# lammps/lammps-plugins

Measured on AMD Instinct MI355X. Metric: Matom-steps/sec, higher is better.
Workload: dtype f64; 1 GPU; REBO-MoS bulk: in.rebomos-bulk cell replicated 24x24x24; atoms=3981312, style=rebomos, parallelism=spatial-dd1, transport=none (one GPU), rccl_library_is_test_double=False, thermo_every=10, displacement_check=every step, deferred on-device flag, dangerous_builds=0, inner_skin=adaptive from 1.0, late_style_list_builds_rank0=0, row_prunings_late_rank0=0, rccl_ranks=1

## Files before the change

lammps-plugins_amd/csrc/domain.hip:

```cpp
#include "mdp_common.h"

#include <rocprim/rocprim.hpp>

#include <cmath>

namespace {

__device__ __forceinline__ void dd_shift_cart(const DdGeom &G, const double s0, const double s1, const double s2,
                                              double out[3])
{
  out[0] = G.h[0] * s0 + G.h[5] * s1 + G.h[4] * s2;
  out[1] = G.h[1] * s1 + G.h[3] * s2;
  out[2] = G.h[2] * s2;
}

__device__ __forceinline__ unsigned dd_cell10(const double u)
{
  int g = (int) (u * 1024.0);
  g = g < 0 ? 0 : (g > 1023 ? 1023 : g);
  return (unsigned) g;
}

template <bool IMAGE>
__global__ __launch_bounds__(256) void dd_remap_kernel(const DdGeom G, const int n, double4 *__restrict__ xq,
// ... 426 lines not shown
  D.nghost_old = c->nghost;
  mdp_tally_drop(c);
  MDP_HIP(c, D.dest.reserve((size_t) n + 1));
  MDP_HIP(c, hipMemsetAsync(D.counters.p, 0, sizeof(int) * (4 * G.nranks + 16), st));
  if (n && c->image_set) dd_remap_kernel<true><<<nblk(n), 256, 0, st>>>(G, n, c->xq.p, D.dest.p, D.counters.p, c->image.p);
  else if (n) dd_remap_kernel<false><<<nblk(n), 256, 0, st>>>(G, n, c->xq.p, D.dest.p, D.counters.p, nullptr);
  MDP_HIP(c, hipGetLastError());
  MDP_TRY(mdp_read_one(c, D.counters.p, sizeof(int) * G.nranks, D.mig_send.data()));
  D.mig_send[G.rank] = 0;
  D.mig_total = 0;
  for (int q = 0; q < G.nranks; q++) D.mig_total += D.mig_send[q];
  if (send_counts)
    for (int q = 0; q < G.nranks; q++) send_counts[q] = D.mig_send[q];
  return MDP_OK;
}

int mdp_dd_migrate_pack(mdp_ctx *c, double *d_buf)
{
  MDP_TRY(dd_require(c));
  MdpDomain &D = c->dd;
  const DdGeom &G = D.G;
  hipStream_t st = c->stream;
  if (!D.mig_total) return MDP_OK;
  if (!d_buf) return mdp_fail(c, MDP_EINVAL, "mdp_dd_migrate_pack: no buffer for %d leaving atoms", D.mig_total);
  std::vector<int> off(2 * (size_t) G.nranks, 0);
  for (int q = 1; q < G.nranks; q++) off[q] = off[q - 1] + D.mig_send[q - 1];
  int *seg = D.counters.p + G.nranks, *cur = D.counters.p + 2 * G.nranks;
  MDP_TRY(mdp_write_small(c, seg, off.data(), sizeof(int) * 2 * G.nranks));
  const int *mask = c->mask_set ? c->mask.p : nullptr;
  if (c->image_set)
    dd_pack_leavers_kernel<true><<<nblk(D.nlocal_old), 256, 0, st>>>(D.nlocal_old, G.rank, D.dest.p, seg, cur, c->xq.p, c->v.p,
                                                                     c->type.p, c->tag.p, mask, c->image.p, d_buf);
  else
    dd_pack_leavers_kernel<false><<<nblk(D.nlocal_old), 256, 0, st>>>(D.nlocal_old, G.rank, D.dest.p, seg, cur, c->xq.p, c->v.p,
                                                                      c->type.p, c->tag.p, mask, nullptr, d_buf);
  MDP_HIP(c, hipGetLastError());
  MDP_HIP(c, hipStreamSynchronize(st));
  return MDP_OK;
}

int mdp_dd_migrate_end(mdp_ctx *c, int narrive, const double *d_buf)
{
  MDP_TRY(dd_require(c));
  MdpDomain &D = c->dd;
  const DdGeom &G = D.G;
  hipStream_t st = c->stream;
  if (narrive < 0 || (narrive > 0 && !d_buf)) return mdp_fail(c, MDP_EINVAL, "mdp_dd_migrate_end: bad arrival buffer");
  const int nold = D.nlocal_old, ntot = nold + narrive, nnew = ntot - D.mig_total;
  if ((long long) ntot >= (1ll << 29)) return mdp_fail(c, MDP_EINVAL, "too many atoms for NEIGHMASK");
  MDP_HIP(c, c->xq.reserve((size_t) ntot + 1, true, st));
  MDP_HIP(c, c->v.reserve((size_t) 3 * ntot + 3, true, st));
  MDP_HIP(c, c->type.reserve((size_t) ntot + 32, true, st));
  MDP_HIP(c, c->tag.reserve((size_t) ntot + 1, true, st));
  MDP_HIP(c, D.dest.reserve((size_t) ntot + 1, true, st));
  if (c->mask_set) MDP_HIP(c, c->mask.reserve((size_t) ntot + 1, true, st));
  if (c->image_set) MDP_HIP(c, c->image.reserve((size_t) ntot + 1, true, st));
  MDP_HIP(c, c->mass_type.reserve(32));
  MDP_HIP(c, hipMemcpyAsync(c->mass_type.p, c->h_mass, sizeof(double) * 16, hipMemcpyHostToDevice, st));
  int *d_map = D.counters.p + 3 * G.nranks;
  MDP_HIP(c, hipMemcpyAsync(d_map, c->map, sizeof(int) * 16, hipMemcpyHostToDevice, st));
  if (narrive)
    dd_unpack_arrivals_kernel<<<nblk(narrive), 256, 0, st>>>(narrive, nold, d_buf, d_map, c->xq.p, c->v.p, c->type.p,
                                                             c->tag.p, c->mask_set ? c->mask.p : nullptr,
                                                             c->image_set ? c->image.p : nullptr, D.dest.p, G.rank);
  MDP_HIP(c, D.key_a.reserve((size_t) ntot + 1));
  MDP_HIP(c, D.key_b.reserve((size_t) ntot + 1));
  MDP_HIP(c, D.idx_a.reserve((size_t) ntot + 1));
  MDP_HIP(c, D.idx_b.reserve((size_t) ntot + 1));
  const size_t room = (size_t) nnew + (size_t) D.nghost_old + (size_t) D.nghost_old / 16;
  MDP_HIP(c, D.xq_tmp.reserve(room + 1));
  MDP_HIP(c, D.v_tmp.reserve((size_t) 3 * nnew + 3));
  MDP_HIP(c, D.type_tmp.reserve(room + 32));
  MDP_HIP(c, D.tag_tmp.reserve(room + 1));
  if (c->mask_set) MDP_HIP(c, D.mask_tmp.reserve((size_t) nnew + 1));
  if (c->image_set) MDP_HIP(c, D.image_tmp.reserve((size_t) nnew + 1));
  MDP_HIP(c, c->rmass.reserve((size_t) nnew + 1));
  if (ntot) {
    const int shell_last = c->cfg.style == 2;
    dd_order_key_kernel<<<nblk(ntot), 256, 0, st>>>(G, ntot, c->xq.p, c->tag.p, D.dest.p, D.key_a.p, D.idx_a.p,
                                                    shell_last);
    MDP_HIP(c, hipGetLastError());
    MDP_TRY(sort_u64(c, D.key_a.p, D.key_b.p, D.idx_a.p, D.idx_b.p, (size_t) ntot, 64));
    if (c->cfg.style == 1) {
      MDP_TRY(mdp_chunk_by_element(c, ntot, nnew, D.idx_b.p, D.idx_a.p, c->xq.p, nullptr, nullptr));
      D.idx_a.swap(D.idx_b);
    }
  }
  if (nnew) {
    dd_permute_kernel<<<nblk(nnew), 256, 0, st>>>(nnew, D.idx_b.p, c->xq.p, c->v.p, c->type.p, c->tag.p, c->mass_type.p,
                                                  D.xq_tmp.p, D.v_tmp.p, D.type_tmp.p, D.tag_tmp.p, c->rmass.p,
                                                  c->mask_set ? c->mask.p : nullptr, c->mask_set ? D.mask_tmp.p : nullptr,
                                                  c->image_set ? c->image.p : nullptr, c->image_set ? D.image_tmp.p : nullptr);
    MDP_HIP(c, hipGetLastError());
  }
  c->xq.swap(D.xq_tmp);
  c->v.swap(D.v_tmp);
  c->type.swap(D.type_tmp);
  c->tag.swap(D.tag_tmp);
  if (c->mask_set) {
    c->mask.swap(D.mask_tmp);
    c->mask_n = nnew;
  }
  if (c->image_set) c->image.swap(D.image_tmp);
  c->nlocal = nnew;
  c->nghost = 0;
  c->nall = nnew;
  c->cfg.nlocal = nnew;
  c->neigh_set = false;
  c->rebo_packed = false;
  return MDP_OK;
}

int mdp_dd_borders_begin(mdp_ctx *c, int *send_counts)
{
  MDP_TRY(dd_require(c));
  MdpDomain &D = c->dd;
  const DdGeom &G = D.G;
  hipStream_t st = c->stream;
  const int n = c->nlocal;
  MDP_HIP(c, D.ent_cnt.reserve((size_t) n + 2));
  MDP_HIP(c, D.ent_off.reserve((size_t) n + 2));
  int nent = 0;
  if (n) {
    dd_border_kernel<false><<<nblk(n), 256, 0, st>>>(G, n, c->xq.p, D.ent_cnt.p, nullptr, nullptr, nullptr, nullptr);
    MDP_HIP(c, hipGetLastError());
    MDP_TRY(mdp_scan_exclusive_int(c, D.ent_cnt.p, D.ent_off.p, n));
    MDP_TRY(mdp_read_one(c, D.ent_off.p + n, sizeof(int), &nent));
  }
  D.nent = nent;
  const int ncls = G.nranks + 1;
  std::vector<int> start(ncls, -1);
  if (nent) {
    MDP_HIP(c, D.ent_atom.reserve((size_t) nent));
    MDP_HIP(c, D.ent_code.reserve((size_t) nent));
    MDP_HIP(c, D.key_a.reserve((size_t) nent));
    MDP_HIP(c, D.key_b.reserve((size_t) nent));
    MDP_HIP(c, D.idx_a.reserve((size_t) nent));
    MDP_HIP(c, D.idx_b.reserve((size_t) nent));
    dd_border_kernel<true><<<nblk(n), 256, 0, st>>>(G, n, c->xq.p, nullptr, D.ent_off.p, D.ent_atom.p, D.ent_code.p,
                                                    D.key_a.p);
    MDP_HIP(c, hipGetLastError());
    MDP_HIP(c, rocprim::transform(rocprim::counting_iterator<int>(0), D.idx_a.p, (size_t) nent,
                                  [] __device__(int v) -> int { return v; }, st));
    int bits = 33;
    while ((1ll << (bits - 32)) < ncls + 1) bits++;
    MDP_TRY(sort_u64(c, D.key_a.p, D.key_b.p, D.idx_a.p, D.idx_b.p, (size_t) nent, bits));
    int *d_start = D.counters.p + 3 * G.nranks + 16;
    MDP_HIP(c, hipMemsetAsync(d_start, 0xFF, sizeof(int) * ncls, st));
    dd_class_start_kernel<<<nblk(nent), 256, 0, st>>>(nent, D.key_b.p, d_start);
    MDP_HIP(c, hipGetLastError());
    MDP_TRY(mdp_read_one(c, d_start, sizeof(int) * ncls, start.data()));
  }
  std::vector<int> cnt(ncls, 0);
  int next = nent;
  for (int k = ncls - 1; k >= 0; k--)
    if (start[k] >= 0) {
      cnt[k] = next - start[k];
      next = start[k];
    }
  D.nself = cnt[0];
  D.nsend = nent - D.nself;
  for (int q = 0; q < G.nranks; q++) D.bord_send[q] = cnt[q + 1];
  if (D.bord_send[G.rank] != 0 && !G.self_remote)
    return mdp_fail(c, MDP_EINVAL, "dd: internal error (self entries in the send list)");
  MDP_HIP(c, c->ghost_owner.reserve((size_t) D.nself + 1));
  MDP_HIP(c, c->ghost_shift.reserve((size_t) 3 * D.nself + 3));
  MDP_HIP(c, D.sendlist.reserve((size_t) D.nsend + 1));
// ... 215 lines not shown
```

lammps-plugins_amd/csrc/mdp_api.hip:

```cpp
#include "mdp_common.h"

#include <rocprim/rocprim.hpp>

#include <condition_variable>
#include <functional>
#include <mutex>
#include <thread>
#include <unistd.h>

#include <cmath>

void mdp_rebomos_fill_dev(mdp_ctx *c, double skin);

int mdp_fail(mdp_ctx *c, int code, const char *fmt, ...)
{
  char buf[1024];
  va_list ap;
  va_start(ap, fmt);
  vsnprintf(buf, sizeof buf, fmt, ap);
  va_end(ap);
  if (c) c->err = buf;
  return code;
}

// ... 502 lines not shown
  nt = nt > W.width() ? W.width() : nt;
  if (nt <= 1) {
    for (size_t k = 0; k < n; k++) dst[k] += src[k];
    return;
  }
  const size_t chunk = ((n + nt - 1) / nt + 7) & ~(size_t) 7;
  W.run(nt, [=](unsigned t) {
    const size_t b = t * chunk, e = b + chunk < n ? b + chunk : n;
    for (size_t k = b; k < e; k++) dst[k] += src[k];
  });
}

int mdp_host_download_add(mdp_ctx *c, double *h_dst, double *h_stage, const double *d_src, size_t n)
{
  hipStream_t st = c->stream;
  size_t cut[MDP_DOWN_CHUNKS + 1];
  int nch = 1;
  cut[0] = 0;
  cut[1] = n;
  if (n > (1u << 21)) {
    const size_t per = ((n + MDP_DOWN_CHUNKS - 1) / MDP_DOWN_CHUNKS + 7) & ~(size_t) 7;
    nch = MDP_DOWN_CHUNKS;
    for (int k = 1; k <= nch; k++) cut[k] = (size_t) k * per < n ? (size_t) k * per : n;
  }
  if (!c->ev_down[0])
    for (int k = 0; k < MDP_DOWN_CHUNKS; k++) MDP_HIP(c, hipEventCreateWithFlags(&c->ev_down[k], hipEventDisableTiming));
  for (int k = 0; k < nch; k++) {
    const size_t b = cut[k], e = cut[k + 1];
    if (b >= e) continue;
    MDP_HIP(c, hipMemcpyAsync(h_stage + b, d_src + b, sizeof(double) * (e - b), hipMemcpyDeviceToHost, st));
    MDP_HIP(c, hipEventRecord(c->ev_down[k], st));
  }
  for (int k = 0; k < nch; k++) {
    const size_t b = cut[k], e = cut[k + 1];
    if (b >= e) continue;
    MDP_HIP(c, hipEventSynchronize(c->ev_down[k]));
    mdp_host_add(h_dst + b, h_stage + b, e - b);
  }
  return MDP_OK;
}

int mdp_pack_xq(mdp_ctx *c, const double *d_x3, const int *d_type, int count)
{
  static_assert(sizeof(double4) == 32, "double4 layout");
  const int n = count >= 0 ? count : c->nall;
  if (n <= 0) return MDP_OK;
  int *d_map = nullptr;
  if (d_type) {
    d_map = c->type.p + c->nall;
  }
  if (c->host_sort)
    pack_xq_perm_kernel<<<nblk(n), 256, 0, c->stream>>>(n, d_x3, d_type, d_map, c->host_perm.p, c->xq.p);
  else
    pack_xq_kernel<<<nblk(n), 256, 0, c->stream>>>(n, d_x3, d_type, d_map, c->xq.p);
  MDP_HIP(c, hipGetLastError());
  return MDP_OK;
}

static int host_sort_atoms(mdp_ctx *c)
{
  const int nall = c->nall;
  const char *e = getenv("MDP_HOST_SORT");
  const bool own_lists = (c->have_rebomos && !c->have_aeam) || (c->have_aeam && c->aeam_device_lists);
  c->host_sort = !c->md && own_lists && c->nlocal > 0 && !(e && atoi(e) == 0) && !c->rebo_host_list;
  if (!c->host_sort) return MDP_OK;
  hipStream_t st = c->stream;
  MDP_HIP(c, c->sort_keys_a.reserve(nall + 1));
  MDP_HIP(c, c->sort_keys_b.reserve(nall + 1));
  MDP_HIP(c, c->cell_of.reserve(nall + 1));
  MDP_HIP(c, c->host_perm.reserve(nall + 1));
  double sc[3];
  for (int d = 0; d < 3; d++) sc[d] = 1024.0 / (c->bbox_hi[d] - c->bbox_lo[d]);
  hilbert_key_kernel<<<nblk(nall), 256, 0, st>>>(nall, c->nlocal, c->xraw.p, c->bbox_lo[0], c->bbox_lo[1],
                                                 c->bbox_lo[2], sc[0], sc[1], sc[2], c->sort_keys_a.p,
                                                 c->cell_of.p);
  MDP_HIP(c, hipGetLastError());
  size_t tmp = 0;
  MDP_HIP(c, rocprim::radix_sort_pairs(nullptr, tmp, c->sort_keys_a.p, c->sort_keys_b.p, c->cell_of.p, c->host_perm.p,
                                       (size_t) nall, 0, 31, st));
  MDP_HIP(c, c->scan_tmp.reserve(tmp + 16));
  MDP_HIP(c, rocprim::radix_sort_pairs(c->scan_tmp.p, tmp, c->sort_keys_a.p, c->sort_keys_b.p, c->cell_of.p,
                                       c->host_perm.p, (size_t) nall, 0, 31, st));
  if (c->have_rebomos && !c->have_aeam) {
    MDP_TRY(mdp_chunk_by_element(c, nall, c->nlocal, c->host_perm.p, c->cell_of.p, nullptr, c->type.p, c->type.p + nall));
    int *p = c->host_perm.p;
    c->host_perm.p = c->cell_of.p;
    c->cell_of.p = p;
    const size_t cp = c->host_perm.cap;
    c->host_perm.cap = c->cell_of.cap;
    c->cell_of.cap = cp;
  }
  return MDP_OK;
}

namespace {
__global__ void chunk_key_kernel(const int n, const int n_owned, const int *__restrict__ idx_in,
                                 const double4 *__restrict__ xq, const int *__restrict__ type,
                                 const int *__restrict__ map, unsigned *__restrict__ key)
{
  const int p = blockIdx.x * 256 + threadIdx.x;
  if (p >= n) return;
  if (p >= n_owned) {
    key[p] = (((unsigned) n_owned >> 5) + 1u) << 1;
    return;
  }
  const int o = idx_in[p];
  int e;
  if (xq)
    e = (int) xq[o].w;
  else {
    const int t = type[o];
    e = map ? map[t] : t - 1;
  }
  key[p] = (((unsigned) p >> 5) << 1) | (e != 0 ? 1u : 0u);
}
}

int mdp_chunk_by_element(mdp_ctx *c, int n, int n_owned, const int *d_idx_in, int *d_idx_out, const double4 *d_xq,
                         const int *d_type, const int *d_map)
{
  if (n <= 0) return MDP_OK;
  MDP_HIP(c, c->sort_keys_a.reserve((size_t) n + 1));
  MDP_HIP(c, c->sort_keys_b.reserve((size_t) n + 1));
  chunk_key_kernel<<<nblk(n), 256, 0, c->stream>>>(n, n_owned, d_idx_in, d_xq, d_type, d_map, c->sort_keys_a.p);
  MDP_HIP(c, hipGetLastError());
  int bits = 2;
  while ((1ull << bits) <= ((((unsigned long long) n_owned >> 5) + 2ull) << 1)) bits++;
  size_t tmp = 0;
  MDP_HIP(c, rocprim::radix_sort_pairs(nullptr, tmp, c->sort_keys_a.p, c->sort_keys_b.p, d_idx_in, d_idx_out, (size_t) n, 0,
                                       bits, c->stream));
  MDP_HIP(c, c->scan_tmp.reserve(tmp + 16));
  MDP_HIP(c, rocprim::radix_sort_pairs(c->scan_tmp.p, tmp, c->sort_keys_a.p, c->sort_keys_b.p, d_idx_in, d_idx_out,
                                       (size_t) n, 0, bits, c->stream));
  return MDP_OK;
}

int mdp_scan_exclusive_int(mdp_ctx *c, const int *d_in, int *d_out, int n)
{
  size_t tmp = 0;
  MDP_HIP(c, rocprim::exclusive_scan(nullptr, tmp, d_in, d_out, 0, (size_t) n + 1, rocprim::plus<int>(), c->stream));
  MDP_HIP(c, c->scan_tmp.reserve(tmp + 16));
  MDP_HIP(c, rocprim::exclusive_scan(c->scan_tmp.p, tmp, d_in, d_out, 0, (size_t) n + 1, rocprim::plus<int>(),
                                     c->stream));
  return MDP_OK;
}

int mdp_scan_exclusive_i64(mdp_ctx *c, const int *d_in, long long *d_out, int n)
{
  size_t tmp = 0;
  auto in = rocprim::make_transform_iterator(d_in, [] __device__(int v) -> long long { return (long long) v; });
  MDP_HIP(c, rocprim::exclusive_scan(nullptr, tmp, in, d_out, 0ll, (size_t) n + 1, rocprim::plus<long long>(),
                                     c->stream));
  MDP_HIP(c, c->scan_tmp.reserve(tmp + 16));
  MDP_HIP(c, rocprim::exclusive_scan(c->scan_tmp.p, tmp, in, d_out, 0ll, (size_t) n + 1, rocprim::plus<long long>(),
                                     c->stream));
  return MDP_OK;
}

extern "C" {

int mdp_abi_version(void) { return MDP_ABI_VERSION; }

int mdp_device_count(void)
{
  int n = 0;
  if (hipGetDeviceCount(&n) != hipSuccess) return 0;
  return n;
}

int mdp_create(mdp_ctx **out, int device)
{
  if (!out) return MDP_EINVAL;
  *out = nullptr;
  int n = 0;
  if (hipGetDeviceCount(&n) != hipSuccess || n <= 0) return MDP_EHIP;
  if (device < 0 || device >= n) return MDP_EINVAL;
  if (hipSetDevice(device) != hipSuccess) return MDP_EHIP;
  mdp_ctx *c = new (std::nothrow) mdp_ctx();
  if (!c) return MDP_ENOMEM;
  c->device = device;
  if (hipStreamCreateWithFlags(&c->stream, hipStreamNonBlocking) != hipSuccess) {
    delete c;
    return MDP_EHIP;
  }
  c->own_stream = true;
  if (c->acc.reserve((size_t) MDP_ACC_STRIDE * (2 + MDP_ACC_SLOTS)) != hipSuccess || c->flags.reserve(8) != hipSuccess ||
      hipHostMalloc((void **) &c->h_pinned, kPinWords * sizeof(double)) != hipSuccess ||
      hipMemset(c->flags.p, 0, 8 * sizeof(int)) != hipSuccess) {
    mdp_destroy(c);
    return MDP_ENOMEM;
  }
  memset(c->map, 0, sizeof c->map);
  memset(c->h_pinned, 0, kPinWords * sizeof(double));
  *out = c;
  return MDP_OK;
}

int mdp_destroy(mdp_ctx *c)
{
  if (!c) return MDP_OK;
  (void) hipSetDevice(c->device);
  if (c->stream) (void) hipStreamSynchronize(c->stream);
  (void) mdp_dd_comm_destroy(c);
  if (c->dd.ev_moved) (void) hipEventDestroy(c->dd.ev_moved);
  host_unregister_all(c);
  for (int k = 0; k < MDP_DOWN_CHUNKS; k++)
    if (c->ev_down[k]) (void) hipEventDestroy(c->ev_down[k]);
  for (int k = 0; k < MDP_UP_RING; k++) {
    if (c->h_up[k]) (void) hipHostFree(c->h_up[k]);
    if (c->ev_up[k]) (void) hipEventDestroy(c->ev_up[k]);
  }
  if (c->h_down) (void) hipHostFree(c->h_down);
  for (int k = 0; k < 2; k++)
    if (c->ev_sflag[k]) (void) hipEventDestroy(c->ev_sflag[k]);
  if (c->h_pinned) (void) hipHostFree(c->h_pinned);
  if (c->h_small) (void) hipHostFree(c->h_small);
  if (c->ev_made)
// ... 415 lines not shown
```

lammps-plugins_amd/csrc/mdp_common.h:

```cpp
#pragma once

#include <hip/hip_runtime.h>

#include <atomic>
#include <cstdarg>
#include <cstdio>
#include <cstdlib>
#include <cstring>
#include <string>
#include <type_traits>
#include <utility>
#include <vector>

#include "devbuf.h"
#include "mdpair_hip.h"

#define MDP_NEIGHMASK 0x1FFFFFFF
#define MDP_CLUSTER 2
static_assert(MDP_CLUSTER == 1 || MDP_CLUSTER == 2, "the Lennard-Jones kernels are instantiated for 1- and 2-atom clusters only");
#define MDP_TILE 16
#define MDP_ACC_SLOTS 512
#define MDP_ACC_STRIDE 16
#define MDP_NOVF_LISTS 7
#define MDP_NCLASS 20
// ... 703 lines not shown
  DevBuf<int> rev16;
  DevBuf<int> ovf;
  int ovf_stride = 0;
  DevBuf<unsigned long long> centre_paths;
  bool centre_full_now = true;
  unsigned long long *centre_cnt_now = nullptr;
  int ovf3_hot[4] = {0, 0, 0, 0};
  DevBuf<mdp_hold_t> xhold_all;
  double skin_inner = 0.0;
  double skin_inner_auto = 1.0;
  double skin_inner_cap = 1.0e9;
  long long computes_since_build = 0;
  bool stale_rebuild = false;
  long long style_builds = 0;
  long long dangerous_builds = 0;
  int sflag_set = 0;
  bool sflag_armed = false;
  bool sflag_committed[2] = {false, false};
  MdpStyleCheck sflag_chk;
  MdpStyleCheckMeta sflag_meta[2];
  hipEvent_t ev_sflag[2] = {nullptr, nullptr};
  MdpNhc nhc;
  MdpLangevin lgv;
  MdpFire fire;
  MdpHeat heat;
  MdpIndent indent;
  MdpSpring spring;
  MdpGforce gforce;
  DevBuf<int> mask;
  bool mask_set = false;
  int mask_n = 0;
  int group_bit = 0, lgv_bit = 0;
  DevBuf<int> image;
  bool image_set = false;
  MdpMsd msd;
  MdpRdf rdf;
  MdpAdf adf;
  MdpCoord coord;
  MdpCentro centro;
  MdpCna cna;
  MdpProfile profile;
  MdpHeatflux heatflux;
  int tally_eflag = -1, tally_vflag = -1;
  bool final_pending = false;
  bool final_deferred_seen = false;
  bool acc_prezeroed = false;
  bool check_now = false;
  DevBuf<double> fnbr;
  DevBuf<double> fown;
  DevBuf<double> vslot;
  DevBuf<char> scan_tmp;

  DevBuf<double> rho, fp;
  DevBuf<int> ang_list;
  DevBuf<int> ang_count;
  int h_ang_count = 0;
  int aeam_cl = 1;
  bool aeam_tiled = false;
  bool aeam_device_lists = false;
  bool skin_set = false;
  bool csr_full = true;
  bool csr_want_full = false;
  int aeam_split = 0;
  bool aeam_ang_remote = false;
  int aeam_phase = 0;
  int aeam_vflag = 0;

  MdpGrid grid;
  double bbox_lo[3] = {0, 0, 0}, bbox_hi[3] = {0, 0, 0};

  bool md = false;
  mdp_md_config cfg;
  DevBuf<double> v;
  DevBuf<mdp_hold_t> xhold;
  DevBuf<double> rmass;
  DevBuf<int> ghost_owner;
  DevBuf<double> ghost_shift;
  DevBuf<double> mass_type;
  double h_mass[16] = {};
  MdpDomain dd;
  DevBuf<int> cell_of, cell_perm, cell_start;
  DevBuf<unsigned> sort_keys_a, sort_keys_b;
  DevBuf<int> sort_vals_b;
  DevBuf<int> nb_cnt;
  double last_eng = 0.0, last_virial[6] = {0, 0, 0, 0, 0, 0};

  bool timing = false;
  hipEvent_t ev[8] = {};
  hipEvent_t ev_sb[8] = {}, ev_se[8] = {};
  unsigned span_mask = 0;
  bool timing_spans = false;
  bool ev_made = false;
  int ev_marks = 0;
  double t_ms[8] = {};
  MdpLedgerScope ledger_close{nullptr};
};

int mdp_fail(mdp_ctx *c, int code, const char *fmt, ...);

enum MdpPin {
  kPinAcc = 0,
  kPinFlags = 16,
  kPinHostCheck = 24,
  kPinMoved = 28,
  kPinSflag = 32,
  kPinOvf = 40,
  kPinGeneral = 44,
  kPinCubic = 45,
  kPinGlob = 46,
  kPinCubicWalk = 47,
  kPinFire = 48,
  kPinWords = 64
};
static_assert(kPinFire + 3 <= kPinWords, "the last pinned word must fit the allocation");
inline int *mdp_pin(const mdp_ctx *c, MdpPin word) { return (int *) (c->h_pinned + word); }

struct MdpStep {
  double dt, dtf, ftm2v;
  const double *mass;
};
inline MdpStep mdp_step(const mdp_ctx *c)
{
  if (c->md) return {c->cfg.dt, 0.5 * c->cfg.dt * c->cfg.ftm2v, c->cfg.ftm2v, c->h_mass};
  return {c->hn_dt, c->hn_dtf, c->hn_ftm2v, c->hn_mass};
}

inline double mdp_margin_scale(const mdp_ctx *c) { return c->md && c->cfg.dt > 0.001 ? c->cfg.dt / 0.001 : 1.0; }

struct MdpRead {
  const void *d_src;
  size_t bytes;
  void *h_dst;
};
int mdp_read_small(mdp_ctx *c, const MdpRead *r, int n);
int mdp_read_one(mdp_ctx *c, const void *d_src, size_t bytes, void *h_dst);
int mdp_write_small(mdp_ctx *c, void *d_dst, const void *h_src, size_t bytes);

#define MDP_HIP(c, call)                                                                             \
  do {                                                                                               \
    hipError_t e_ = (call);                                                                          \
    if (e_ != hipSuccess)                                                                            \
      return mdp_fail((c), MDP_EHIP, "%s:%d: %s -> %s", __FILE__, __LINE__, #call, hipGetErrorString(e_)); \
  } while (0)

#define MDP_TRY(expr)                                                                                \
  do {                                                                                               \
    int rc_ = (expr);                                                                                \
    if (rc_ != MDP_OK) return rc_;                                                                   \
  } while (0)

template <typename... P, typename... A>
inline int mdp_launch(mdp_ctx *c, void (*kernel)(P...), int grid, int block, size_t lds, hipStream_t st, A &&...args)
{
  if (lds > 48 * 1024)
    MDP_HIP(c, hipFuncSetAttribute((const void *) kernel, hipFuncAttributeMaxDynamicSharedMemorySize, (int) lds));
  kernel<<<grid, block, lds, st>>>(std::forward<A>(args)...);
  MDP_HIP(c, hipGetLastError());
  return MDP_OK;
}

template <class F> inline int mdp_with_bool(const bool b, F &&f) { return b ? f(std::true_type{}) : f(std::false_type{}); }

struct MdpRows {
  const int *len, *split;
  const unsigned short *lj16;
};
inline MdpRows mdp_rows(const mdp_ctx *c)
{
  if (c->prune_valid) return {c->lj_len_in.p, c->lj_split_in.p, c->lj16_in.p};
  return {nullptr, c->lj_split.p, c->lj16.p};
}
inline void mdp_rows_renewed(mdp_ctx *c)
{
  c->prune_valid = false;
  c->prune_stale = false;
  c->prune_epoch++;
}

inline bool aeam_wants_tiles(const mdp_ctx *c)
{
  const char *e = getenv("MDP_AEAM_TILE");
  return (c->md || c->aeam_device_lists) && !(e && atoi(e) == 0) && c->aeam.ntypes <= MDP_AEAM_MAXT;
}

int mdp_pack_xq(mdp_ctx *c, const double *d_x3, const int *d_type_or_null, int count = -1);
int mdp_rebomos_host_precheck(mdp_ctx *c);
int mdp_host_ghost_scalar(mdp_ctx *c, double *d_a);
int mdp_host_ghost_fold(mdp_ctx *c, int w, double *d_a);
int mdp_hold(mdp_ctx *c, int n, mdp_hold_t *d_hold);
int mdp_moved(mdp_ctx *c, int n, int max_grid, double trigsq, double hardsq, const mdp_hold_t *d_hold, int *flag,
              const mdp_hold_t *d_prune = nullptr, double ptrigsq = 0.0, double phardsq = 0.0);
int mdp_scan_exclusive_int(mdp_ctx *c, const int *d_in, int *d_out, int n);
int mdp_chunk_by_element(mdp_ctx *c, int n, int n_owned, const int *d_idx_in, int *d_idx_out, const double4 *d_xq,
                         const int *d_type, const int *d_map);
int mdp_scan_exclusive_i64(mdp_ctx *c, const int *d_in, long long *d_out, int n);
int mdp_rebomos_repack(mdp_ctx *c);
int mdp_prune_upkeep(mdp_ctx *c, const double cut[4], double skin, bool own_check, bool may_prune, bool *due);
int mdp_tile_rows_build(mdp_ctx *c, const RebomosDev &P, int cl, bool from_csr, const MdpRead *ride, bool *ok);
int mdp_tile_lists_build(mdp_ctx *c, const double cutsq[4], int cl, bool *ok);
int mdp_rebomos_run(mdp_ctx *c, int eflag, int vflag, bool zero_f);
int mdp_rebomos_run_begin(mdp_ctx *c, int eflag, int vflag);
int mdp_rebomos_run_end(mdp_ctx *c, int eflag, int vflag);
int mdp_aeam_prepare(mdp_ctx *c);
int mdp_aeam_run_begin(mdp_ctx *c, int eflag, int vflag);
int mdp_aeam_run_density(mdp_ctx *c, int eflag);
int mdp_aeam_run_force_begin(mdp_ctx *c, int eflag, int vflag);
int mdp_aeam_run_force(mdp_ctx *c, int eflag, int vflag);
int mdp_md_build_master_list(mdp_ctx *c);
int mdp_md_build_neighbors_impl(mdp_ctx *c);
int mdp_bin_atoms(mdp_ctx *c, double cutoff, const double lo[3], const double hi[3]);
void mdp_time_mark(mdp_ctx *c, int k);
void mdp_span_begin(mdp_ctx *c, int k);
void mdp_span_end(mdp_ctx *c, int k);
int mdp_host_pinned_reserve(mdp_ctx *c, size_t ndoubles);
int mdp_host_upload(mdp_ctx *c, void *d_dst, const void *h_src, size_t bytes);
int mdp_host_refresh_ghosts(mdp_ctx *c);
int mdp_md_advance(mdp_ctx *c, bool with_final, int *flag, double trigsq, double hardsq);
int mdp_md_ghost_fold(mdp_ctx *c, int w, double *d_a);
int mdp_md_flush_final(mdp_ctx *c);
int mdp_moved_take(mdp_ctx *c, int *moved, int *dangerous);
int *mdp_moved_arm(mdp_ctx *c, double skin, double *trigsq, double *hardsq);
int mdp_moved_post(mdp_ctx *c, bool borrow_sflag);
int mdp_nhc_open(mdp_ctx *c, bool with_final, const double **vscale);
int mdp_nhc_final(mdp_ctx *c);
template <int NB> int mdp_lgv_open(mdp_ctx *c, bool with_final, bool initial, bool *apply, MdpLgvArgs<NB> *L);
template <int NB> int mdp_lgv_close(mdp_ctx *c, const MdpLgvArgs<NB> &L);
int mdp_group_args(mdp_ctx *c, bool *masked, MdpGroupArgs *M);
int mdp_lgv_check_disjoint(mdp_ctx *c, const char *who);
int mdp_heat_pass(mdp_ctx *c);
inline void mdp_heat_count_step(mdp_ctx *c)
{
  if (!c->heat.on) return;
  c->heat.step++;
  c->heat.started = true;
}
int mdp_heat_mask(mdp_ctx *c, const char *who);
int mdp_heat_check(mdp_ctx *c);
int mdp_gforce_mask(mdp_ctx *c, const char *who);
int mdp_indent_pass(mdp_ctx *c);
int mdp_spring_pass(mdp_ctx *c);
int mdp_gforce_pass(mdp_ctx *c);
enum MdpStageId { kStageIndent = 0, kStageSpring, kStageGforce, kStageCount };
struct MdpStage {
  MdpPostForce &(*base)(mdp_ctx *);
  int (*pass)(mdp_ctx *);
  const char *api, *many, *one;
};
inline constexpr MdpStage kMdpStages[kStageCount] = {
    {[](mdp_ctx *c) -> MdpPostForce & { return c->indent; }, mdp_indent_pass, "mdp_indent", "indenters", "indenter"},
    {[](mdp_ctx *c) -> MdpPostForce & { return c->spring; }, mdp_spring_pass, "mdp_spring", "springs", "spring"},
    {[](mdp_ctx *c) -> MdpPostForce & { return c->gforce; }, mdp_gforce_pass, "mdp_gforce", "group forces", "group force"},
};
inline int mdp_postforce_apply(mdp_ctx *c, int through = kStageCount - 1)
{
  for (int s = 0; s <= through; s++) {
    MdpPostForce &h = kMdpStages[s].base(c);
    if (!h.on || h.applied) continue;
    MDP_TRY(kMdpStages[s].pass(c));
    h.applied = true;
  }
  return MDP_OK;
}
inline void mdp_postforce_count_step(mdp_ctx *c)
{
  for (const MdpStage &s : kMdpStages) {
    MdpPostForce &h = s.base(c);
    if (!h.on) continue;
    h.nhalf++;
    h.applied = false;
  }
}
enum MdpRefuse { kRefuseOffFirst, kRefuseOneRank };
int mdp_postforce_refuse_setup(mdp_ctx *c, int s);
int mdp_postforce_commit(mdp_ctx *c, int s, int words, int n, const int *groupbit, void *cfg_dst, const void *cfg, size_t cfg_bytes);
int mdp_postforce_run(mdp_ctx *c, int s, long long first);
int mdp_postforce_state(mdp_ctx *c, int s, int k, int len, double *out);
int mdp_postforce_off(mdp_ctx *c, int s);
// ... 97 lines not shown
```

Baseline: 1574 Matom-steps/s.

## Order atoms into same-element groups of eight with nearest-partner pairing

Replaces the per-32-atom element chunking sort with a scan-based placement. Owned atoms are split by element into groups of eight, groups are interleaved four at a time, and each group is reordered so that consecutive pairs are spatial nearest partners. This tightens the neighbor-list unions for the two-atom clusters that share tile rows, so padded row work in the REBO kernels should shrink. It adds several small kernels and two scans at reorder time, and the old path stays available through an environment variable.

```diff
diff --git a/lammps-plugins_amd/csrc/domain.hip b/lammps-plugins_amd/csrc/domain.hip
--- a/lammps-plugins_amd/csrc/domain.hip
+++ b/lammps-plugins_amd/csrc/domain.hip
@@ -532,7 +532,7 @@
     MDP_HIP(c, hipGetLastError());
     MDP_TRY(sort_u64(c, D.key_a.p, D.key_b.p, D.idx_a.p, D.idx_b.p, (size_t) ntot, 64));
     if (c->cfg.style == 1) {
-      MDP_TRY(mdp_chunk_by_element(c, ntot, nnew, D.idx_b.p, D.idx_a.p, c->xq.p, nullptr, nullptr));
+      MDP_TRY(mdp_order_pairs(c, ntot, nnew, D.idx_b.p, D.idx_a.p, c->xq.p, nullptr, nullptr, nullptr));
       D.idx_a.swap(D.idx_b);
     }
   }
diff --git a/lammps-plugins_amd/csrc/mdp_api.hip b/lammps-plugins_amd/csrc/mdp_api.hip
--- a/lammps-plugins_amd/csrc/mdp_api.hip
+++ b/lammps-plugins_amd/csrc/mdp_api.hip
@@ -608,7 +608,7 @@
   MDP_HIP(c, rocprim::radix_sort_pairs(c->scan_tmp.p, tmp, c->sort_keys_a.p, c->sort_keys_b.p, c->cell_of.p,
                                        c->host_perm.p, (size_t) nall, 0, 31, st));
   if (c->have_rebomos && !c->have_aeam) {
-    MDP_TRY(mdp_chunk_by_element(c, nall, c->nlocal, c->host_perm.p, c->cell_of.p, nullptr, c->type.p, c->type.p + nall));
+    MDP_TRY(mdp_order_pairs(c, nall, c->nlocal, c->host_perm.p, c->cell_of.p, nullptr, c->xraw.p, c->type.p, c->type.p + nall));
     int *p = c->host_perm.p;
     c->host_perm.p = c->cell_of.p;
     c->cell_of.p = p;
@@ -620,6 +620,138 @@
 }
 
 namespace {
+__device__ __forceinline__ int order_element(const int o, const double4 *__restrict__ xq, const int *__restrict__ type,
+                                             const int *__restrict__ map)
+{
+  if (xq) return (int) xq[o].w != 0;
+  const int t = type[o];
+  return (map ? map[t] : t - 1) != 0;
+}
+
+__global__ __launch_bounds__(256) void pair_flag_kernel(const int n_owned, const int *__restrict__ idx_in,
+                                                        const double4 *__restrict__ xq, const int *__restrict__ type,
+                                                        const int *__restrict__ map, int *__restrict__ flag)
+{
+  const int p = blockIdx.x * 256 + threadIdx.x;
+  if (p > n_owned) return;
+  flag[p] = p < n_owned ? order_element(idx_in[p], xq, type, map) : 0;
+}
+
+struct PairRank {
+  int e, rank, complete;
+};
+__device__ __forceinline__ PairRank pair_rank(const int p, const int n_owned, const int *__restrict__ flag,
+                                              const int *__restrict__ before)
+{
+  PairRank r;
+  const int n1 = before[n_owned], b = before[p];
+  r.e = flag[p];
+  r.rank = r.e ? b : p - b;
+  r.complete = (r.rank | 7) < (r.e ? n1 : n_owned - n1);
+  return r;
+}
+
+__global__ __launch_bounds__(256) void pair_lead_kernel(const int n_owned, const int *__restrict__ flag,
+                                                        const int *__restrict__ before, int *__restrict__ lead)
+{
+  const int p = blockIdx.x * 256 + threadIdx.x;
+  if (p > n_owned) return;
+  int l = 0;
+  if (p < n_owned) {
+    const PairRank r = pair_rank(p, n_owned, flag, before);
+    l = r.complete && (r.rank & 7) == 0;
+  }
+  lead[p] = l;
+}
+
+__global__ __launch_bounds__(256) void pair_slot_kernel(const int n_owned, const int gstride, const int *__restrict__ flag,
+                                                        const int *__restrict__ before, const int *__restrict__ lead_before,
+                                                        int *__restrict__ slot, int *__restrict__ slot_el)
+{
+  const int p = blockIdx.x * 256 + threadIdx.x;
+  if (p >= n_owned) return;
+  const PairRank r = pair_rank(p, n_owned, flag, before);
+  if (r.complete && (r.rank & 7) == 0) {
+    const int s = lead_before[p];
+    slot[r.e * gstride + (r.rank >> 3)] = s;
+    slot_el[s] = r.e;
+  }
+}
+
+__global__ __launch_bounds__(256) void pair_place_kernel(const int n, const int n_owned, const int gstride,
+                                                         const int *__restrict__ idx_in, const int *__restrict__ flag,
+                                                         const int *__restrict__ before, const int *__restrict__ lead_before,
+                                                         const int *__restrict__ slot, const int *__restrict__ slot_el,
+                                                         int *__restrict__ idx_out)
+{
+  const int p = blockIdx.x * 256 + threadIdx.x;
+  if (p >= n) return;
+  int dst = p;
+  if (p < n_owned) {
+    const PairRank r = pair_rank(p, n_owned, flag, before);
+    const int ngroups = lead_before[n_owned];
+    if (r.complete) {
+      const int s = slot[r.e * gstride + (r.rank >> 3)], t4 = s & ~3;
+      int first = 0, same_ahead = 0;
+      for (int k = t4; k < t4 + 4 && k < ngroups; k++) {
+        const int ek = slot_el[k];
+        first += ek == 0;
+        same_ahead += k < s && ek == r.e;
+      }
+      dst = 8 * (t4 + (r.e ? first : 0) + same_ahead) + (r.rank & 7);
+    } else
+      dst = 8 * ngroups + (r.e ? (n_owned - before[n_owned]) & 7 : 0) + (r.rank & 7);
+  }
+  idx_out[dst] = idx_in[p];
+}
+
+__global__ __launch_bounds__(256) void pair_partner_kernel(const int max_groups, const int *__restrict__ ngroups,
+                                                           const double4 *__restrict__ xq, const double *__restrict__ x3,
+                                                           int *__restrict__ idx)
+{
+  const int g = blockIdx.x * 256 + threadIdx.x;
+  if (g >= max_groups || g >= *ngroups) return;
+  int id[8];
+  double x[8], y[8], z[8], dc[8];
+#pragma unroll
+  for (int k = 0; k < 8; k++) {
+    const int o = id[k] = idx[8 * (size_t) g + k];
+    if (xq) {
+      const double4 q = xq[o];
+      x[k] = q.x, y[k] = q.y, z[k] = q.z;
+    } else
+      x[k] = x3[3 * (size_t) o], y[k] = x3[3 * (size_t) o + 1], z[k] = x3[3 * (size_t) o + 2];
+  }
+  double cx = x[0], cy = y[0], cz = z[0];
+#pragma unroll
+  for (int k = 1; k < 8; k++) cx = __dadd_rn(cx, x[k]), cy = __dadd_rn(cy, y[k]), cz = __dadd_rn(cz, z[k]);
+  cx *= 0.125, cy *= 0.125, cz *= 0.125;
+  auto dist2 = [](double dx, double dy, double dz) {
+    return __dadd_rn(__dadd_rn(__dmul_rn(dx, dx), __dmul_rn(dy, dy)), __dmul_rn(dz, dz));
+  };
+#pragma unroll
+  for (int k = 0; k < 8; k++) dc[k] = dist2(x[k] - cx, y[k] - cy, z[k] - cz);
+  unsigned used = 0;
+  int out[8];
+  for (int t = 0; t < 4; t++) {
+    int a = -1, b = -1;
+    double da = 0.0, db = 0.0;
+    for (int k = 0; k < 8; k++)
+      if (!(used >> k & 1) && (a < 0 || dc[k] > da)) a = k, da = dc[k];
+    used |= 1u << a;
+    for (int k = 0; k < 8; k++)
+      if (!(used >> k & 1)) {
+        const double d = dist2(x[k] - x[a], y[k] - y[a], z[k] - z[a]);
+        if (b < 0 || d < db) b = k, db = d;
+      }
+    used |= 1u << b;
+    out[2 * t] = id[a];
+    out[2 * t + 1] = id[b];
+  }
+#pragma unroll
+  for (int k = 0; k < 8; k++) idx[8 * (size_t) g + k] = out[k];
+}
+
 __global__ void chunk_key_kernel(const int n, const int n_owned, const int *__restrict__ idx_in,
                                  const double4 *__restrict__ xq, const int *__restrict__ type,
                                  const int *__restrict__ map, unsigned *__restrict__ key)
@@ -642,10 +774,35 @@
 }
 }
 
-int mdp_chunk_by_element(mdp_ctx *c, int n, int n_owned, const int *d_idx_in, int *d_idx_out, const double4 *d_xq,
-                         const int *d_type, const int *d_map)
-{
-  if (n <= 0) return MDP_OK;
+static int order_groups_of_eight(mdp_ctx *c, int n, int n_owned, const int *d_idx_in, int *d_idx_out, const double4 *d_xq,
+                                 const double *d_x3, const int *d_type, const int *d_map)
+{
+  hipStream_t st = c->stream;
+  const int gstride = n_owned / 8 + 1;
+  MDP_HIP(c, c->sort_keys_a.reserve((size_t) n_owned + 1));
+  MDP_HIP(c, c->sort_keys_b.reserve((size_t) n_owned + 1));
+  MDP_HIP(c, c->pair_lead.reserve((size_t) n_owned + 1));
+  MDP_HIP(c, c->pair_lead_before.reserve((size_t) n_owned + 1));
+  MDP_HIP(c, c->pair_slot.reserve((size_t) 3 * gstride));
+  int *flag = (int *) c->sort_keys_a.p, *before = (int *) c->sort_keys_b.p;
+  MDP_TRY(mdp_launch(c, pair_flag_kernel, nblk(n_owned + 1), 256, 0, st, n_owned, d_idx_in, d_xq, d_type, d_map, flag));
+  MDP_TRY(mdp_scan_exclusive_int(c, flag, before, n_owned));
+  MDP_TRY(mdp_launch(c, pair_lead_kernel, nblk(n_owned + 1), 256, 0, st, n_owned, flag, before, c->pair_lead.p));
+  MDP_TRY(mdp_scan_exclusive_int(c, c->pair_lead.p, c->pair_lead_before.p, n_owned));
+  if (n_owned)
+    MDP_TRY(mdp_launch(c, pair_slot_kernel, nblk(n_owned), 256, 0, st, n_owned, gstride, flag, before,
+                       c->pair_lead_before.p, c->pair_slot.p, c->pair_slot.p + 2 * (size_t) gstride));
+  MDP_TRY(mdp_launch(c, pair_place_kernel, nblk(n), 256, 0, st, n, n_owned, gstride, d_idx_in, flag, before,
+                     c->pair_lead_before.p, c->pair_slot.p, c->pair_slot.p + 2 * (size_t) gstride, d_idx_out));
+  if (n_owned / 8)
+    MDP_TRY(mdp_launch(c, pair_partner_kernel, nblk(n_owned / 8), 256, 0, st, n_owned / 8, c->pair_lead_before.p + n_owned,
+                       d_xq, d_x3, d_idx_out));
+  return MDP_OK;
+}
+
+static int order_runs_of_32(mdp_ctx *c, int n, int n_owned, const int *d_idx_in, int *d_idx_out, const double4 *d_xq,
+                            const int *d_type, const int *d_map)
+{
   MDP_HIP(c, c->sort_keys_a.reserve((size_t) n + 1));
   MDP_HIP(c, c->sort_keys_b.reserve((size_t) n + 1));
   chunk_key_kernel<<<nblk(n), 256, 0, c->stream>>>(n, n_owned, d_idx_in, d_xq, d_type, d_map, c->sort_keys_a.p);
@@ -659,6 +816,15 @@
   MDP_HIP(c, rocprim::radix_sort_pairs(c->scan_tmp.p, tmp, c->sort_keys_a.p, c->sort_keys_b.p, d_idx_in, d_idx_out,
                                        (size_t) n, 0, bits, c->stream));
   return MDP_OK;
+}
+
+int mdp_order_pairs(mdp_ctx *c, int n, int n_owned, const int *d_idx_in, int *d_idx_out, const double4 *d_xq,
+                    const double *d_x3, const int *d_type, const int *d_map)
+{
+  if (n <= 0) return MDP_OK;
+  const char *e = getenv("MDP_PAIR_ORDER");
+  if (e && atoi(e) == 0) return order_runs_of_32(c, n, n_owned, d_idx_in, d_idx_out, d_xq, d_type, d_map);
+  return order_groups_of_eight(c, n, n_owned, d_idx_in, d_idx_out, d_xq, d_x3, d_type, d_map);
 }
 
 int mdp_scan_exclusive_int(mdp_ctx *c, const int *d_in, int *d_out, int n)
diff --git a/lammps-plugins_amd/csrc/mdp_common.h b/lammps-plugins_amd/csrc/mdp_common.h
--- a/lammps-plugins_amd/csrc/mdp_common.h
+++ b/lammps-plugins_amd/csrc/mdp_common.h
@@ -809,6 +809,7 @@
   DevBuf<int> cell_of, cell_perm, cell_start;
   DevBuf<unsigned> sort_keys_a, sort_keys_b;
   DevBuf<int> sort_vals_b;
+  DevBuf<int> pair_lead, pair_lead_before, pair_slot;
   DevBuf<int> nb_cnt;
   double last_eng = 0.0, last_virial[6] = {0, 0, 0, 0, 0, 0};
 
@@ -918,8 +919,8 @@
 int mdp_moved(mdp_ctx *c, int n, int max_grid, double trigsq, double hardsq, const mdp_hold_t *d_hold, int *flag,
               const mdp_hold_t *d_prune = nullptr, double ptrigsq = 0.0, double phardsq = 0.0);
 int mdp_scan_exclusive_int(mdp_ctx *c, const int *d_in, int *d_out, int n);
-int mdp_chunk_by_element(mdp_ctx *c, int n, int n_owned, const int *d_idx_in, int *d_idx_out, const double4 *d_xq,
-                         const int *d_type, const int *d_map);
+int mdp_order_pairs(mdp_ctx *c, int n, int n_owned, const int *d_idx_in, int *d_idx_out, const double4 *d_xq,
+                    const double *d_x3, const int *d_type, const int *d_map);
 int mdp_scan_exclusive_i64(mdp_ctx *c, const int *d_in, long long *d_out, int n);
 int mdp_rebomos_repack(mdp_ctx *c);
 int mdp_prune_upkeep(mdp_ctx *c, const double cut[4], double skin, bool own_check, bool may_prune, bool *due);
diff --git a/profiles/pair_order/model.py b/profiles/pair_order/model.py
--- /dev/null
+++ b/profiles/pair_order/model.py
@@ -0,0 +1,155 @@
+#!/usr/bin/env python3
+import argparse
+import importlib.util
+import os
+import sys
+
+import numpy as np
+from scipy.spatial import cKDTree
+
+ROOT = os.path.dirname(os.path.dirname(os.path.dirname(os.path.abspath(__file__))))
+
+
+def _system_module():
+    spec = importlib.util.spec_from_file_location("mdp_system", os.path.join(ROOT, "lammps-plugins_amd", "host", "system.py"))
+    mod = importlib.util.module_from_spec(spec)
+    sys.modules["mdp_system"] = mod
+    spec.loader.exec_module(mod)
+    return mod
+
+
+def lj_cut():
+    v = []
+    for line in open(os.path.join(ROOT, "tests", "golden", "potentials", "MoS.REBO.set5b")):
+        t = line.split("#")[0].split()
+        if t:
+            v.append(float(t[0]))
+    sm, ss = v[59], v[60]
+    return 2.5 * np.array([[sm, (sm + ss) / 2], [(sm + ss) / 2, ss]])
+
+
+def hilbert30(c):
+    X = [c[:, d].astype(np.uint32).copy() for d in range(3)]
+    Q = np.uint32(1 << 9)
+    while Q > 1:
+        P = np.uint32(Q - 1)
+        for d in range(3):
+            hit = (X[d] & Q) != 0
+            t = np.where(hit, np.uint32(0), (X[0] ^ X[d]) & P)
+            X[0] = np.where(hit, X[0] ^ P, X[0] ^ t)
+            if d:
+                X[d] = X[d] ^ t
+        Q = np.uint32(Q >> 1)
+    X[1] ^= X[0]
+    X[2] ^= X[1]
+    t = np.zeros_like(X[0])
+    Q = np.uint32(1 << 9)
+    while Q > 1:
+        t = np.where((X[2] & Q) != 0, t ^ np.uint32(Q - 1), t)
+        Q = np.uint32(Q >> 1)
+    X = [x ^ t for x in X]
+    key = np.zeros(len(c), dtype=np.uint64)
+    for b in range(9, -1, -1):
+        for d in range(3):
+            key = (key << np.uint64(1)) | ((X[d] >> np.uint32(b)) & np.uint32(1)).astype(np.uint64)
+    return key
+
+
+def runs_by_element(el, run):
+    p = np.arange(len(el))
+    return np.lexsort((p, el, p // run))
+
+
+def partner_rule(x):
+    dc = ((x - x.mean(axis=0)) ** 2).sum(axis=1)
+    left, order = list(range(8)), []
+    while left:
+        a = max(left, key=lambda k: (dc[k], -k))
+        left.remove(a)
+        b = min(left, key=lambda k: (((x[k] - x[a]) ** 2).sum(), k))
+        left.remove(b)
+        order += [a, b]
+    return order
+
+
+def groups_of_eight(el, x, key="first", partners=False):
+    groups, tail = [], []
+    for e in (0, 1):
+        idx = np.flatnonzero(el == e)
+        full = 8 * (len(idx) // 8)
+        groups.append(idx[:full].reshape(-1, 8))
+        tail.append(idx[full:])
+    g = np.concatenate(groups)
+    k = g[:, 0] if key == "first" else g.mean(axis=1)
+    g = g[np.lexsort((g[:, 0], k))]
+    g = g[np.lexsort((np.arange(len(g)), el[g[:, 0]], np.arange(len(g)) // 4))]
+    if partners:
+        g = np.array([row[partner_rule(x[row])] for row in g])
+    return np.concatenate([g.ravel()] + tail)
+
+
+ORDERINGS = [
+    ("runs of 32 by element (MDP_PAIR_ORDER=0)", lambda el, x: runs_by_element(el, 32)),
+    ("runs of 96 by element", lambda el, x: runs_by_element(el, 96)),
+    ("groups of 8, merged on the first member", lambda el, x: groups_of_eight(el, x)),
+    ("... plus nearest partners (the device's rule)", lambda el, x: groups_of_eight(el, x, partners=True)),
+    ("groups of 8 + partners, merged on the mean position", lambda el, x: groups_of_eight(el, x, "mean", True)),
+]
+
+
+def main():
+    ap = argparse.ArgumentParser(description=__doc__, formatter_class=argparse.RawDescriptionHelpFormatter)
+    ap.add_argument("--replicate", type=int, default=5)
+    ap.add_argument("--jitter", type=float, default=0.0)
+    ap.add_argument("--seed", type=int, default=3)
+    ap.add_argument("--buffer", type=float, default=0.3)
+    ap.add_argument("--tiles", type=int, default=160, help="tiles in the sample")
+    a = ap.parse_args()
+    S = _system_module()
+    s = S.replicate(S.rebomos_bulk_cell(), (a.replicate,) * 3)
+    if a.jitter > 0:
+        s = S.jitter(s, a.jitter, a.seed)
+    x = S.wrap(s.box, s.x)
+    cut = lj_cut() + a.buffer
+    owner, shift = S.make_ghosts(s.box, x, float(cut.max()))
+    x_all = np.concatenate([x, x[owner] + S.mul_upper(shift, s.box.h)])
+    el_all = np.concatenate([s.type, s.type[owner]]) - 1
+    tree = cKDTree(x_all)
+    cell = np.clip((s.box.x2lamda(x) * 1024.0).astype(np.int64), 0, 1023)
+    curve = np.lexsort((s.tag, hilbert30(cell)))
+    el_c, x_c = el_all[curve], x[curve]
+    ntile = s.n // 32
+    sample = np.sort(np.random.default_rng(1).choice(ntile, size=min(a.tiles, ntile), replace=False))
+    print(f"REBO-MoS bulk {a.replicate}^3: {s.n} atoms, jitter {a.jitter} A (seed {a.seed}), window + {a.buffer} A, "
+          f"{len(sample)} of {ntile} tiles")
+    print(f"{'ordering':52s} {'one atom':>8s} {'union':>7s} {'wave-max':>8s} {'+ pad':>7s} {'ratio':>6s}  tile union mean / max")
+    base = None
+    for name, fn in ORDERINGS:
+        atom = curve[fn(el_c, x_c)]
+        alone, union, wmax, wpad, tun = [], [], [], [], []
+        for t in sample:
+            ids = atom[32 * t:32 * t + 32]
+            near = tree.query_ball_point(x[ids], float(cut.max()))
+            segs = []
+            for i, nb in zip(ids, near):
+                nb = np.array(nb)
+                nb = nb[nb != i]
+                d = np.linalg.norm(x_all[nb] - x[i], axis=1)
+                ok = d <= cut[el_all[i], el_all[nb]]
+                segs.append([set(nb[ok & (el_all[nb] == e)].tolist()) for e in (0, 1)])
+                alone.append(sum(len(q) for q in segs[-1]))
+            rows = np.array([[len(segs[2 * k][e] | segs[2 * k + 1][e]) for e in (0, 1)] for k in range(16)])
+            union += rows.sum(axis=1).tolist()
+            for w in range(4):
+                m = rows[4 * w:4 * w + 4].max(axis=0)
+                wmax += [int(m.sum())] * 4
+                wpad += [int((16 * -(-m // 16)).sum())] * 4
+            tun.append(len(set().union(*(q for sg in segs for q in sg))))
+        res = [float(np.mean(v)) for v in (alone, union, wmax, wpad)]
+        base = base or res[3]
+        print(f"{name:52s} {res[0]:8.1f} {res[1]:7.1f} {res[2]:8.1f} {res[3]:7.1f} {res[3] / base:6.3f}  "
+              f"{np.mean(tun):6.0f} / {max(tun)}")
+
+
+if __name__ == "__main__":
+    main()
```

Measured after the change: 1595 Matom-steps/s, median of 6. 1.3% higher.
